# linyicheng1/trackingBench-SLAM

Measured on AMD Instinct MI355X. Metric: frames/sec end-to-end (extract+match+local-BA), higher is better.
Workload: dtype u8 (pyramid/FAST/ORB/Hamming) + f64 (pose-opt/BA); 1 GPU; 1280x720 stereo, 8-level pyramid x0.8, 2000 kpts/image (FAST 80/30), searchByBF L<->R, pose-opt, 10-KF/5000-pt local BA x10 iters; distinct_synthetic_pairs=64, distinct_ba_windows=32, ba_partitions=3, ba_schedule=joined at the end of every step, parallelism=frames sharded x1, RCCL gather of tracks

## Files before the change

### trackingbench_slam_amd/csrc/k_pyramid.hip

```cpp
#include "tb_internal.h"
#include "tb_device.h"

__global__ void __launch_bounds__(256)
k_resize(PlanGeom g, uint8_t* __restrict__ slab, const ResizeX* __restrict__ rx, const ResizeY* __restrict__ ry,
         int level) {
    const int b = blockIdx.y;
    const LevelGeom& D = g.lv[level];
    const int groupsPerRow = D.stride >> 2;
    const int group = blockIdx.x * blockDim.x + threadIdx.x;
    if (group >= groupsPerRow * D.h) return;
    const int dy = group / groupsPerRow;
    const int dx0 = (group - dy * groupsPerRow) << 2;

    int sstride;
    const uint8_t* src = tb_level_ptr(g, slab, b, level - 1, &sstride);
    uint8_t* dst = slab + (size_t)b * g.slabBytes + D.off + (size_t)dy * D.stride;

    const ResizeY yy = ry[dy];
    const uint8_t* S0 = src + (size_t)yy.sy0 * sstride;
    const uint8_t* S1 = src + (size_t)yy.sy1 * sstride;
    const int b0 = yy.b0, b1 = yy.b1;
    uint32_t packed = 0;
#pragma unroll
    for (int i = 0; i < 4; i++) {
        const int dx = dx0 + i;
        if (dx < D.w) {
            const ResizeX xx = rx[dx];
            const int r0 = S0[xx.sx] * xx.a0 + S0[xx.sx1] * xx.a1;
            const int r1 = S1[xx.sx] * xx.a0 + S1[xx.sx1] * xx.a1;
            int v = (((b0 * (r0 >> 4)) >> 16) + ((b1 * (r1 >> 4)) >> 16) + 2) >> 2;
            v = min(max(v, 0), 255);
            packed |= (uint32_t)v << (8 * i);
        }
    }
    *reinterpret_cast<uint32_t*>(dst + dx0) = packed;
}

#define RS_ROWS 8
#define RS_MAXR 14

__global__ void __launch_bounds__(64)
k_resize_lds(PlanGeom g, uint8_t* __restrict__ slab, const ResizeX* __restrict__ rx, const ResizeY* __restrict__ ry,
             int level, int rowBytes, int nImages, int by_image, int tilesX, int tilesY) {
    extern __shared__ __attribute__((aligned(16))) uint8_t rows[];
    int b, tx, ty;
    if (by_image) {
        const unsigned L = blockIdx.x, j = L >> 3, T = (unsigned)(tilesX * tilesY), grp = j / T, t = j - grp * T;
        b = (int)(grp * 8u + (L & 7u));
        if (b >= nImages) return;
        ty = (int)(t / (unsigned)tilesX); tx = (int)(t - (unsigned)ty * (unsigned)tilesX);
    } else {
        b = blockIdx.z; tx = blockIdx.x; ty = blockIdx.y;
    }
    const int dy0 = ty * RS_ROWS, lane = threadIdx.x;
    const LevelGeom& D = g.lv[level];
    const int X0 = tx * 256;
    int sstride;
    const uint8_t* src = tb_level_ptr(g, slab, b, level - 1, &sstride);
    const int dy1 = min(dy0 + RS_ROWS, D.h) - 1;
    const int xl = min(X0 + 255, D.w - 1);
    const int sxa = rx[X0].sx & ~3, sxb = rx[xl].sx1;
    const int ndw = ((sxb - sxa) >> 2) + 1;
    const int sya = ry[dy0].sy0, syb = ry[dy1].sy1;
    const int nrows = syb - sya + 1;
    if (nrows <= RS_MAXR && ndw <= 128) {
        uint32_t v[RS_MAXR][2];
        const uint8_t* S = src + (size_t)sya * sstride + sxa + 4 * lane;
#pragma unroll
        for (int r = 0; r < RS_MAXR; r++) {
            v[r][0] = (r < nrows && lane < ndw) ? *reinterpret_cast<const uint32_t*>(S + (size_t)r * sstride) : 0u;
            v[r][1] = (r < nrows && lane + 64 < ndw) ? *reinterpret_cast<const uint32_t*>(S + (size_t)r * sstride + 256) : 0u;
        }
#pragma unroll
        for (int r = 0; r < RS_MAXR; r++) {
            if (r < nrows && lane < ndw) *reinterpret_cast<uint32_t*>(rows + r * rowBytes + 4 * lane) = v[r][0];
            if (r < nrows && lane + 64 < ndw) *reinterpret_cast<uint32_t*>(rows + r * rowBytes + 4 * lane + 256) = v[r][1];
        }
    } else {
        for (int r = 0; r < nrows; r++) {
            const uint8_t* S = src + (size_t)(sya + r) * sstride + sxa;
            for (int dd = lane; dd < ndw; dd += 64)
                *reinterpret_cast<uint32_t*>(rows + r * rowBytes + 4 * dd) = *reinterpret_cast<const uint32_t*>(S + 4 * dd);
        }
    }
    __syncthreads();
    const int dx0 = X0 + 4 * lane;
    if (dx0 >= D.stride) return;
    int o0[4], o1[4], a0[4], a1[4];
#pragma unroll
    for (int i = 0; i < 4; i++) {
        const int dx = min(dx0 + i, D.w - 1);
        const ResizeX xx = rx[dx];
        o0[i] = xx.sx - sxa; o1[i] = xx.sx1 - sxa; a0[i] = xx.a0; a1[i] = xx.a1;
    }
    auto hrow = [&](int sy, int (&hh)[4]) {
        const uint8_t* R = rows + (sy - sya) * rowBytes;
#pragma unroll
        for (int i = 0; i < 4; i++) hh[i] = (R[o0[i]] * a0[i] + R[o1[i]] * a1[i]) >> 4;
    };
    auto emit = [&](int dy, int b0, int b1, const int (&h0)[4], const int (&h1)[4]) {
        uint32_t packed = 0;
#pragma unroll
        for (int i = 0; i < 4; i++)
            if (dx0 + i < D.w) packed |= (uint32_t)((((b0 * h0[i]) >> 16) + ((b1 * h1[i]) >> 16) + 2) >> 2) << (8 * i);
        *reinterpret_cast<uint32_t*>(slab + (size_t)b * g.slabBytes + D.off + (size_t)dy * D.stride + dx0) = packed;
    };
    for (int dy = dy0; dy <= dy1; dy += 2) {
        const ResizeY ya = ry[dy];
        int hA[4], hB[4];
        hrow(ya.sy0, hA);
        hrow(ya.sy1, hB);
        emit(dy, ya.b0, ya.b1, hA, hB);
        if (dy + 1 <= dy1) {
            const ResizeY yb = ry[dy + 1];
            int hC[4];
            if (yb.sy0 == ya.sy1) {
                hrow(yb.sy1, hC);
                emit(dy + 1, yb.b0, yb.b1, hB, hC);
            } else {
                hrow(yb.sy0, hA);
                hrow(yb.sy1, hC);
                emit(dy + 1, yb.b0, yb.b1, hA, hC);
            }
        }
    }
}

int tbk_resize_level(tb_extractor* ex, int level, int n) {
    tb_ctx* ctx = ex->ctx;
    const LevelGeom& D = ex->g.lv[level];
    const LevelGeom& Sg = ex->g.lv[level - 1];
    const bool ext0 = (level - 1 == 0) && ex->g.img0 != nullptr;
    const int sstride = ext0 ? ex->g.img0_stride : Sg.stride;
    const uintptr_t sbase = ext0 ? reinterpret_cast<uintptr_t>(ex->g.img0) : 0;
    const unsigned long long spitch = ext0 ? ex->g.img0_pitch : 0;
    const bool aligned = (sstride % 4 == 0) && (sbase % 4 == 0) && (spitch % 4 == 0) && (sstride >= ((Sg.w + 3) & ~3));
    const double rx_ratio = (double)Sg.w / (double)D.w, ry_ratio = (double)Sg.h / (double)D.h;
    const int rowBytes = (((int)(256.0 * rx_ratio) + 16 + 3) & ~3) + 4;
    const int srows = (int)(RS_ROWS * ry_ratio) + 3;
    const size_t lds = (size_t)rowBytes * srows;
    if (aligned && lds <= 48 * 1024) {
        const int tilesX = (D.stride + 255) / 256, tilesY = (D.h + RS_ROWS - 1) / RS_ROWS;
        const int by_image = n >= 64 ? 1 : 0;
        const dim3 grid = by_image ? dim3((unsigned)(tilesX * tilesY) * 8u * (unsigned)((n + 7) / 8)) : dim3(tilesX, tilesY, n);
        return tb_launch(ctx, "k_resize", k_resize_lds, grid, dim3(64), lds, ex->g, ex->d_slab, ex->d_rx[level], ex->d_ry[level], level,
                         rowBytes, n, by_image, tilesX, tilesY);
    }
    const int groups = (D.stride >> 2) * D.h;
    dim3 grid((groups + 255) / 256, n);
    return tb_launch(ctx, "k_resize", k_resize, grid, dim3(256), 0, ex->g, ex->d_slab, ex->d_rx[level], ex->d_ry[level], level);
}

typedef unsigned int tb_u4 __attribute__((ext_vector_type(4)));
__global__ void __launch_bounds__(256)
k_copy16(const tb_u4* __restrict__ src, tb_u4* __restrict__ dst, size_t n16) {
    const size_t i0 = (size_t)blockIdx.x * 1024 + threadIdx.x;
    tb_u4 v[4];
#pragma unroll
    for (int k = 0; k < 4; k++) v[k] = (i0 + 256 * k < n16) ? __builtin_nontemporal_load(src + i0 + 256 * k) : (tb_u4){0, 0, 0, 0};
#pragma unroll
    for (int k = 0; k < 4; k++)
        if (i0 + 256 * k < n16) __builtin_nontemporal_store(v[k], dst + i0 + 256 * k);
}

int tbk_copy16(tb_ctx* ctx, const void* d_src, void* d_dst, size_t bytes) {
    const size_t n16 = bytes / 16;
    if (n16 == 0) return TB_OK;
    const unsigned blocks = (unsigned)((n16 + 1023) / 1024);
    return tb_launch(ctx, nullptr, k_copy16, dim3(blocks), dim3(256), 0, (const tb_u4*)d_src, (tb_u4*)d_dst, n16);
}

__global__ void __launch_bounds__(256)
k_pack_rows(const uint8_t* __restrict__ src, int row_bytes, int cap, const int32_t* __restrict__ counts, int nframes,
            uint8_t* __restrict__ dst, long long* __restrict__ total_out) {
    __shared__ long long red[4];
    const int f = blockIdx.x, tid = threadIdx.x;
    long long before = 0, all = 0;
    for (int i = tid; i < nframes; i += 256) {
        const long long c = min(max(counts[i], 0), cap);
        all += c;
        if (i < f) before += c;
    }
    for (int pass = 0; pass < 2; pass++) {
        long long v = pass == 0 ? before : all;
#pragma unroll
        for (int d = 32; d > 0; d >>= 1) v += __shfl_xor(v, d, 64);
        __syncthreads();
        if ((tid & 63) == 0) red[tid >> 6] = v;
        __syncthreads();
        v = red[0] + red[1] + red[2] + red[3];
        if (pass == 0) before = v; else all = v;
    }
    if (f == 0 && tid == 0 && total_out) total_out[0] = all;
    const int n = min(max(counts[f], 0), cap);
    const size_t nb = (size_t)n * row_bytes;
    const uint32_t* s4 = reinterpret_cast<const uint32_t*>(src + (size_t)f * cap * row_bytes);
    uint32_t* d4 = reinterpret_cast<uint32_t*>(dst + (size_t)before * row_bytes);
    for (size_t i = tid; i < nb / 4; i += 256) d4[i] = s4[i];
}

int tbk_pack_rows(tb_ctx* ctx, const void* d_src, int row_bytes, int cap, const int32_t* d_counts, int nframes, void* d_dst, long long* d_total) {
    if (nframes <= 0) return TB_OK;
    return tb_launch(ctx, nullptr, k_pack_rows, dim3(nframes), dim3(256), 0, (const uint8_t*)d_src, row_bytes, cap, d_counts, nframes,
                     (uint8_t*)d_dst, d_total);
}
```

Measured before the change: 33910 frames/s.

## Stage resize source tile with 128-bit buffer loads and flattened row/segment indexing

```diff
diff --git a/trackingbench_slam_amd/csrc/k_pyramid.hip b/trackingbench_slam_amd/csrc/k_pyramid.hip
--- a/trackingbench_slam_amd/csrc/k_pyramid.hip
+++ b/trackingbench_slam_amd/csrc/k_pyramid.hip
@@ -37,11 +37,14 @@
 }
 
 #define RS_ROWS 8
-#define RS_MAXR 14
-
+#define RS_NLD 6
+
+typedef unsigned int rs_u4 __attribute__((ext_vector_type(4)));
+
+template <bool WIDE>
 __global__ void __launch_bounds__(64)
 k_resize_lds(PlanGeom g, uint8_t* __restrict__ slab, const ResizeX* __restrict__ rx, const ResizeY* __restrict__ ry,
-             int level, int rowBytes, int nImages, int by_image, int tilesX, int tilesY) {
+             int level, int rowBytes, int srows, unsigned recip, int nImages, int by_image, int tilesX, int tilesY) {
     extern __shared__ __attribute__((aligned(16))) uint8_t rows[];
     int b, tx, ty;
     if (by_image) {
@@ -52,6 +55,7 @@
     } else {
         b = blockIdx.z; tx = blockIdx.x; ty = blockIdx.y;
     }
+    constexpr int U = WIDE ? 16 : 4;
     const int dy0 = ty * RS_ROWS, lane = threadIdx.x;
     const LevelGeom& D = g.lv[level];
     const int X0 = tx * 256;
@@ -59,68 +63,92 @@
     const uint8_t* src = tb_level_ptr(g, slab, b, level - 1, &sstride);
     const int dy1 = min(dy0 + RS_ROWS, D.h) - 1;
     const int xl = min(X0 + 255, D.w - 1);
-    const int sxa = rx[X0].sx & ~3, sxb = rx[xl].sx1;
-    const int ndw = ((sxb - sxa) >> 2) + 1;
-    const int sya = ry[dy0].sy0, syb = ry[dy1].sy1;
-    const int nrows = syb - sya + 1;
-    if (nrows <= RS_MAXR && ndw <= 128) {
-        uint32_t v[RS_MAXR][2];
-        const uint8_t* S = src + (size_t)sya * sstride + sxa + 4 * lane;
-#pragma unroll
-        for (int r = 0; r < RS_MAXR; r++) {
-            v[r][0] = (r < nrows && lane < ndw) ? *reinterpret_cast<const uint32_t*>(S + (size_t)r * sstride) : 0u;
-            v[r][1] = (r < nrows && lane + 64 < ndw) ? *reinterpret_cast<const uint32_t*>(S + (size_t)r * sstride + 256) : 0u;
+    const int sxa = rx[min(X0, D.w - 1)].sx & ~(U - 1), sxb = rx[xl].sx1;
+    ResizeY yy[RS_ROWS];
+#pragma unroll
+    for (int k = 0; k < RS_ROWS; k++) yy[k] = ry[min(dy0 + k, dy1)];
+    const int sya = yy[0].sy0;
+    const int S = rowBytes / U;
+    const int nrows = min(yy[RS_ROWS - 1].sy1 - sya + 1, srows);
+    const int total = nrows * S;
+    const int nseg = min((sxb - sxa) / U + 1, S);
+    {
+        const int rowEnd = (g.lv[level - 1].w + U - 1) & ~(U - 1);
+        const __amdgpu_buffer_rsrc_t rs = __builtin_amdgcn_make_buffer_rsrc(
+            const_cast<uint8_t*>(src) + (size_t)sya * sstride + sxa, 0, (nrows - 1) * sstride + rowEnd - sxa, 0x00020000);
+        for (int i0 = 0; i0 < total; i0 += 64 * RS_NLD) {
+            if constexpr (WIDE) {
+                rs_u4 v[RS_NLD];
+#pragma unroll
+                for (int k = 0; k < RS_NLD; k++) {
+                    const unsigned idx = (unsigned)(i0 + 64 * k + lane), row = (idx * recip) >> 22, seg = idx - row * (unsigned)S;
+                    v[k] = __builtin_amdgcn_raw_buffer_load_b128(rs, seg < (unsigned)nseg ? (int)row * sstride + U * (int)seg : 0x7ffffff0, 0, 0);
+                }
+#pragma unroll
+                for (int k = 0; k < RS_NLD; k++) {
+                    const int idx = i0 + 64 * k + lane;
+                    if (idx < total) *reinterpret_cast<rs_u4*>(rows + U * idx) = v[k];
+                }
+            } else {
+                uint32_t v[RS_NLD];
+#pragma unroll
+                for (int k = 0; k < RS_NLD; k++) {
+                    const unsigned idx = (unsigned)(i0 + 64 * k + lane), row = (idx * recip) >> 22, seg = idx - row * (unsigned)S;
+                    v[k] = __builtin_amdgcn_raw_buffer_load_b32(rs, seg < (unsigned)nseg ? (int)row * sstride + U * (int)seg : 0x7ffffff0, 0, 0);
+                }
+#pragma unroll
+                for (int k = 0; k < RS_NLD; k++) {
+                    const int idx = i0 + 64 * k + lane;
+                    if (idx < total) *reinterpret_cast<uint32_t*>(rows + U * idx) = v[k];
+                }
+            }
         }
-#pragma unroll
-        for (int r = 0; r < RS_MAXR; r++) {
-            if (r < nrows && lane < ndw) *reinterpret_cast<uint32_t*>(rows + r * rowBytes + 4 * lane) = v[r][0];
-            if (r < nrows && lane + 64 < ndw) *reinterpret_cast<uint32_t*>(rows + r * rowBytes + 4 * lane + 256) = v[r][1];
-        }
-    } else {
-        for (int r = 0; r < nrows; r++) {
-            const uint8_t* S = src + (size_t)(sya + r) * sstride + sxa;
-            for (int dd = lane; dd < ndw; dd += 64)
-                *reinterpret_cast<uint32_t*>(rows + r * rowBytes + 4 * dd) = *reinterpret_cast<const uint32_t*>(S + 4 * dd);
-        }
-    }
+    }
+    const int dx0 = X0 + 4 * lane;
+    int o0[4], o1[4];
+    uint32_t a0[4], a1[4];
+#pragma unroll
+    for (int i = 0; i < 4; i++) {
+        const ResizeX xx = rx[min(dx0 + i, D.w - 1)];
+        o0[i] = xx.sx - sxa; o1[i] = xx.sx1 - sxa; a0[i] = (uint32_t)xx.a0; a1[i] = (uint32_t)xx.a1;
+    }
+    const int nkeep = min(max(D.w - dx0, 0), 4);
+    const uint32_t keep = nkeep >= 4 ? 0xffffffffu : ((1u << (8 * nkeep)) - 1u);
+    const __amdgpu_buffer_rsrc_t rd = __builtin_amdgcn_make_buffer_rsrc(
+        slab + (size_t)b * g.slabBytes + D.off + (size_t)dy0 * D.stride + X0, 0, (dy1 - dy0 + 1) * D.stride - X0, 0x00020000);
+    const uint32_t doff = dx0 < D.stride ? 4u * lane : 0x7ffffff0u;
     __syncthreads();
-    const int dx0 = X0 + 4 * lane;
-    if (dx0 >= D.stride) return;
-    int o0[4], o1[4], a0[4], a1[4];
-#pragma unroll
-    for (int i = 0; i < 4; i++) {
-        const int dx = min(dx0 + i, D.w - 1);
-        const ResizeX xx = rx[dx];
-        o0[i] = xx.sx - sxa; o1[i] = xx.sx1 - sxa; a0[i] = xx.a0; a1[i] = xx.a1;
-    }
-    auto hrow = [&](int sy, int (&hh)[4]) {
+    auto hrow = [&](int sy, uint32_t (&hh)[4]) {
         const uint8_t* R = rows + (sy - sya) * rowBytes;
 #pragma unroll
-        for (int i = 0; i < 4; i++) hh[i] = (R[o0[i]] * a0[i] + R[o1[i]] * a1[i]) >> 4;
+        for (int i = 0; i < 4; i++) hh[i] = (__umul24(R[o0[i]], a0[i]) + __umul24(R[o1[i]], a1[i])) >> 4;
     };
-    auto emit = [&](int dy, int b0, int b1, const int (&h0)[4], const int (&h1)[4]) {
-        uint32_t packed = 0;
-#pragma unroll
-        for (int i = 0; i < 4; i++)
-            if (dx0 + i < D.w) packed |= (uint32_t)((((b0 * h0[i]) >> 16) + ((b1 * h1[i]) >> 16) + 2) >> 2) << (8 * i);
-        *reinterpret_cast<uint32_t*>(slab + (size_t)b * g.slabBytes + D.off + (size_t)dy * D.stride + dx0) = packed;
+    auto emit = [&](int k, int b0, int b1, const uint32_t (&h0)[4], const uint32_t (&h1)[4]) {
+        const uint32_t B0 = (uint32_t)b0 << 16, B1 = (uint32_t)b1 << 16;
+        uint32_t v[4];
+#pragma unroll
+        for (int i = 0; i < 4; i++) v[i] = (__umulhi(h0[i], B0) + __umulhi(h1[i], B1) + 2u) >> 2;
+        const uint32_t packed = (v[0] | (v[1] << 8)) | ((v[2] | (v[3] << 8)) << 16);
+        __builtin_amdgcn_raw_buffer_store_b32(packed & keep, rd, (int)((uint32_t)(k * D.stride) + doff), 0, 0);
     };
-    for (int dy = dy0; dy <= dy1; dy += 2) {
-        const ResizeY ya = ry[dy];
-        int hA[4], hB[4];
+#pragma unroll
+    for (int k = 0; k < RS_ROWS; k += 2) {
+        if (dy0 + k > dy1) break;
+        const ResizeY ya = yy[k];
+        uint32_t hA[4], hB[4];
         hrow(ya.sy0, hA);
         hrow(ya.sy1, hB);
-        emit(dy, ya.b0, ya.b1, hA, hB);
-        if (dy + 1 <= dy1) {
-            const ResizeY yb = ry[dy + 1];
-            int hC[4];
+        emit(k, ya.b0, ya.b1, hA, hB);
+        if (dy0 + k + 1 <= dy1) {
+            const ResizeY yb = yy[k + 1];
+            uint32_t hC[4];
             if (yb.sy0 == ya.sy1) {
                 hrow(yb.sy1, hC);
-                emit(dy + 1, yb.b0, yb.b1, hB, hC);
+                emit(k + 1, yb.b0, yb.b1, hB, hC);
             } else {
                 hrow(yb.sy0, hA);
                 hrow(yb.sy1, hC);
-                emit(dy + 1, yb.b0, yb.b1, hA, hC);
+                emit(k + 1, yb.b0, yb.b1, hA, hC);
             }
         }
     }
@@ -135,16 +163,20 @@
     const uintptr_t sbase = ext0 ? reinterpret_cast<uintptr_t>(ex->g.img0) : 0;
     const unsigned long long spitch = ext0 ? ex->g.img0_pitch : 0;
     const bool aligned = (sstride % 4 == 0) && (sbase % 4 == 0) && (spitch % 4 == 0) && (sstride >= ((Sg.w + 3) & ~3));
+    const bool wide = aligned && (sstride % 16 == 0) && (sbase % 16 == 0) && (spitch % 16 == 0) && (sstride >= ((Sg.w + 15) & ~15));
     const double rx_ratio = (double)Sg.w / (double)D.w, ry_ratio = (double)Sg.h / (double)D.h;
-    const int rowBytes = (((int)(256.0 * rx_ratio) + 16 + 3) & ~3) + 4;
+    const int rowBytes = ((int)ceil(255.0 * rx_ratio) + 2 + 15 + 15) & ~15;
     const int srows = (int)(RS_ROWS * ry_ratio) + 3;
     const size_t lds = (size_t)rowBytes * srows;
-    if (aligned && lds <= 48 * 1024) {
+    const long long S = rowBytes / (wide ? 16 : 4);
+    const bool divides = (srows * S + 64 * RS_NLD) * S < (1ll << 22) && srows < 512;
+    if (aligned && lds <= 48 * 1024 && divides) {
         const int tilesX = (D.stride + 255) / 256, tilesY = (D.h + RS_ROWS - 1) / RS_ROWS;
         const int by_image = n >= 64 ? 1 : 0;
         const dim3 grid = by_image ? dim3((unsigned)(tilesX * tilesY) * 8u * (unsigned)((n + 7) / 8)) : dim3(tilesX, tilesY, n);
-        return tb_launch(ctx, "k_resize", k_resize_lds, grid, dim3(64), lds, ex->g, ex->d_slab, ex->d_rx[level], ex->d_ry[level], level,
-                         rowBytes, n, by_image, tilesX, tilesY);
+        const unsigned recip = (unsigned)((1u << 22) / (unsigned)S + 1u);
+        return tb_launch(ctx, "k_resize", wide ? k_resize_lds<true> : k_resize_lds<false>, grid, dim3(64), lds, ex->g, ex->d_slab,
+                         ex->d_rx[level], ex->d_ry[level], level, rowBytes, srows, recip, n, by_image, tilesX, tilesY);
     }
     const int groups = (D.stride >> 2) * D.h;
     dim3 grid((groups + 255) / 256, n);
```

Result: faster. 34290 frames/s, median of 6 (+1.1%).
